# lzc452/SSL-VIT-VIDEO-ANALYTICS

Hardware: AMD Instinct MI355X
Metric: clips/sec (8x3x224x224) MAE ViT-Tiny pretrain, 1/2/4/8 GPU + recon-loss parity (higher is better)
Workload: dtype bf16; 1 GPU; BASELINE config 2: TinyViT-21M-variant MAE (stem+stages 1-3) + 4x384 decoder, T=8, 224x224, mask 0.75, bf16 autocast; model=tiny_vit_21m_variant + TinyVideoMAE, global_batch=256, per_gpu_batch=256, frames=8, image_size=224, parallelism=dp1

## Files before the change

include/sm_api.h:

```cpp
#ifndef SM_API_H
#define SM_API_H
#include <stdint.h>
#include <hip/hip_runtime_api.h>

#ifdef __cplusplus
extern "C" {
#endif

int64_t sm_gemm_workspace_bytes(int ab_dtype, int M, int N, int K);
int sm_gemm(int ab_dtype, int c_dtype, int a_layout, int b_layout, int M, int N, int K,
            const void* A, int64_t lda, const void* B, int64_t ldb, void* C, int64_t ldc,
            const float* bias, float alpha, float beta, int epi, void* aux, const void* R,
            float drop_p, uint64_t seed, const float* row_scale, int64_t rows_per_group,
            void* workspace, int64_t ws_bytes, hipStream_t stream);
int sm_gemm_persistent(int mode);
int sm_gemm_tuning(int key, int set, int value, int* prev);
int64_t sm_linear_dw_bias_workspace_bytes(int rows, int nout, int nin);
int sm_linear_dw_bias(int rows, int nout, int nin, const void* dy, const void* x, float* dW, float* db,
                      int accumulate, void* ws, int64_t ws_bytes, hipStream_t stream);
int sm_linear_dx_gelu(int M, int N, int K, const void* dy, const void* w, const void* pre, void* dx, void* h,
                      float drop_p, uint64_t seed, hipStream_t stream);
int sm_linear_dw_bias_gelu(int rows, int nout, int nin, const void* dy, const void* pre, float drop_p,
                           uint64_t seed, float* dW, float* db, int accumulate, void* ws, int64_t ws_bytes,
                           hipStream_t stream);
// ... 7 lines not shown
int sm_linear_bnin(int M, int N, int K, const void* a, const float* a_mean, const float* a_rstd,
                   const float* a_w, const float* a_b, const void* w, void* y, hipStream_t stream);
int sm_linear_bnin_bn_stats(int M, int N, int K, const void* a, const float* a_mean, const float* a_rstd,
                            const float* a_w, const float* a_b, const void* w, void* y, float* mean,
                            float* rstd, float* run_mean, float* run_var, int64_t* num_batches_tracked,
                            float momentum, float eps, int updates, void* ws, int64_t ws_bytes,
                            hipStream_t stream);
int sm_bn_apply_res_bn(int x_dtype, int y_dtype, int64_t M, int C, const void* x, const float* mean,
                       const float* rstd, const float* w, const float* b, void* y, int gelu, const void* R,
                       const float* r_mean, const float* r_rstd, const float* r_w, const float* r_b,
                       const float* row_scale, int64_t rows_per_group, hipStream_t st);
int64_t sm_linear_dw_se_workspace_bytes(int rows, int nout, int nin);
int sm_linear_dw_se(int rows, int nout, int nin, const void* dy, const void* a2, const float* act_mean,
                    const float* act_rstd, const float* act_w, const float* act_b, int act_gelu, const float* gate,
                    int hw, float* dW, int accumulate, void* ws, int64_t ws_bytes, hipStream_t stream);

int sm_attn_fwd(int dtype, int N, int L, int H, int D, const void* qkv, void* out, float* lse,
                float scale, float drop_p, uint64_t seed, hipStream_t st);
int64_t sm_attn_bwd_workspace_bytes(int dtype, int N, int L, int H, int D);
int sm_attn_bwd(int dtype, int N, int L, int H, int D, const void* qkv, const void* o,
                const void* dout, const float* lse, float* delta_ws, void* dqkv,
                float scale, float drop_p, uint64_t seed, hipStream_t st);
int sm_attn_tuning(int key, int set, int value, int* prev);

int sm_layernorm_fwd(int x_dtype, int y_dtype, int64_t M, int C, const void* x, const float* gamma,
                     const float* beta, void* y, float* mean, float* rstd, float eps, hipStream_t st);
int64_t sm_layernorm_bwd_workspace_bytes(int64_t M, int C);
int sm_layernorm_bwd(int x_dtype, int dy_dtype, int dx_dtype, int64_t M, int C, const void* dy,
                     const void* x, const float* mean, const float* rstd, const float* gamma,
                     void* dx, const void* dres, float* dgamma, float* dbeta, void* ws,
// ... 74 lines not shown
                        const float* w, void* y, float* part, hipStream_t st);
int64_t sm_dwconv_fused_bwd_workspace_bytes(int F, int H, int W, int C, int stride);
int sm_dwconv_fused_bwd(int F, int H, int W, int C, int stride, const void* dy, const void* x,
                        const float* in_mean, const float* in_rstd, const float* in_w, const float* in_b,
                        int in_gelu, const float* w, void* dx, float* dw, void* ws, int64_t ws_bytes,
                        hipStream_t st);
int64_t sm_dwconv_bn_bwd_workspace_bytes(int F, int H, int W, int C);
int sm_dwconv_bn_bwd(int F, int H, int W, int C, const void* dy, const void* x, const float* bn_mean,
                     const float* bn_rstd, const float* bn_w, const float* bn_b, int bn_gelu, const float* w,
                     void* dx, float* dw, float* dgamma, float* dbeta, void* ws, int64_t ws_bytes,
                     hipStream_t st);
int sm_dwconv_s2_bn_bwd(int F, int H, int W, int C, const void* dy, const void* x, const float* bn_mean,
                        const float* bn_rstd, const float* bn_w, const float* bn_b, int bn_gelu, const float* w,
                        void* dx, float* dw, float* dgamma, float* dbeta, void* ws, int64_t ws_bytes,
                        hipStream_t st);
int sm_dwconv_bwd(int dtype, const void* dy, const void* x, const float* w, void* dx, float* dw, int F,
                  int H, int W, int C, int stride, void* ws, int64_t ws_bytes, hipStream_t st);

int64_t sm_se_workspace_bytes(int F, int HW, int C);
int sm_se_fwd(int dtype, const void* x, const float* act_mean, const float* act_rstd, const float* act_w,
              const float* act_b, int act_gelu, int F, int HW, int C, int R, const float* w1, const float* w2,
              float* pooled, float* z1, float* s, void* y, void* ws, int64_t ws_bytes, hipStream_t st);
int sm_se_bwd(int dtype, const void* dy, const void* x, const float* act_mean, const float* act_rstd,
              const float* act_w, const float* act_b, int act_gelu, int F, int HW, int C, int R,
              const float* w1, const float* w2, const float* s, const float* z1, float* dz2, float* dz1,
              void* dx, void* ws, int64_t ws_bytes, hipStream_t st);
int sm_se_scale(int dtype, const void* x, const float* act_mean, const float* act_rstd, const float* act_w,
                const float* act_b, int act_gelu, const float* s, void* y, int F, int HW, int C, hipStream_t st);
int64_t sm_se_bn_bwd_workspace_bytes(int F, int HW, int C);
int sm_se_bn_bwd(int dtype, const void* dy, const void* x, const float* bn_mean, const float* bn_rstd,
// ... 52 lines not shown
```

ssl-vit-video-analytics_amd/csrc/conv.hip:

```cpp
#include <algorithm>

#include "common.h"
#include "sm_api.h"

namespace {

inline int ew_blocks(int64_t n) {
  int64_t b = (n + 255) / 256;
  if (b > 16384) b = 16384;
  return b < 1 ? 1 : (int)b;
}

struct ClipView {
  const float* p;
  int B, T, H, W;
  int64_t sB, sC, sT, sH, sW;
};

template <typename TO>
__global__ void stem_im2col_kernel(ClipView v, int Ho, int Wo, int stride, TO* col ) {
  const int64_t P = (int64_t)v.B * v.T * Ho * Wo;
  for (int64_t i = blockIdx.x * (int64_t)blockDim.x + threadIdx.x; i < P; i += (int64_t)gridDim.x * blockDim.x) {
    const int xo = (int)(i % Wo);
    const int64_t r = i / Wo;
// ... 1852 lines not shown
  else
    hipLaunchKernelGGL((dwf_wgrad_kernel<2>), g2, dim3(256), lds, st, (const __bf16*)dy, (const __bf16*)x, act, part,
                       H, W, C, Ho, Wo, dwf_remap());
  colred(part, F, C * 9, nullptr, dw, 1, st);
  SM_CHECK_LAUNCH();
  return 0;
}

extern "C" int64_t sm_dwconv_bn_bwd_workspace_bytes(int F, int H, int W, int C) {
  return ((int64_t)F * C * 9 + (int64_t)F * 2 * C + 2 * C) * 4 + 2 * C * 8 + 64;
}

static int dwconv_bn_bwd(int stride, int F, int H, int W, int C, const void* dy, const void* x, const float* bn_mean,
                         const float* bn_rstd, const float* bn_w, const float* bn_b, int bn_gelu, const float* w,
                         void* dx, float* dw, float* dgamma, float* dbeta, void* ws, int64_t ws_bytes,
                         hipStream_t st) {
  if (bad_stride(stride)) return -2;
  const int Ho = (H + 2 - 3) / stride + 1, Wo = (W + 2 - 3) / stride + 1;
  size_t lds = stride == 1 ? dwf_lds_bytes(W, 1) + DWB_PAD + 4 * DWF_CB * 4
                           : (size_t)DwRing<1, DWB2_TYO>::NR * (Wo + 2) * 64 + DWB2_PAD + 13 * DWF_CB * 4;
  if (lds < 256 * 4 * 4) lds = 256 * 4 * 4;
  if (!dwf_shape_ok(F, W, C, stride) || !bn_mean || !dx || lds > 64 * 1024) return -2;
  if (stride == 2 && DwRing<1, DWB2_TYO>::NEW * Wo * 4 > 256 * DWF_KV) return -2;
  if (((uintptr_t)x & 15) || ((uintptr_t)dy & 15) || ((uintptr_t)dx & 15) || C / 8 > 256) return -2;
  if (ws_bytes < sm_dwconv_bn_bwd_workspace_bytes(F, H, W, C)) return -4;
  float* part_w = (float*)ws;
  float* part_bn = part_w + (int64_t)F * C * 9;
  float* coef = part_bn + (int64_t)F * 2 * C;
  double* sums = (double*)(((uintptr_t)(coef + 2 * C) + 7) & ~(uintptr_t)7);
  ChanAffine bn{bn_mean, bn_rstd, bn_w, bn_b, bn_gelu};
  const dim3 grid((C / DWF_CB) * F);
  if (stride == 2) {
    const bool rag = W % DWB2_PX != 0;
    if (bn_gelu && !rag)
      hipLaunchKernelGGL((dwb2_kernel<true, false>), grid, dim3(256), lds, st, (const __bf16*)dy, (const __bf16*)x, bn,
                         w, (__bf16*)dx, part_w, part_bn, H, W, C, Ho, Wo, dwf_remap());
    else if (bn_gelu)
      hipLaunchKernelGGL((dwb2_kernel<true, true>), grid, dim3(256), lds, st, (const __bf16*)dy, (const __bf16*)x, bn,
                         w, (__bf16*)dx, part_w, part_bn, H, W, C, Ho, Wo, dwf_remap());
    else
      hipLaunchKernelGGL((dwb2_kernel<false, true>), grid, dim3(256), lds, st, (const __bf16*)dy, (const __bf16*)x, bn,
                         w, (__bf16*)dx, part_w, part_bn, H, W, C, Ho, Wo, dwf_remap());
  } else {
    if (bn_gelu)
      hipLaunchKernelGGL((dwb_kernel<true, true>), grid, dim3(256), lds, st, (const __bf16*)dy, (const __bf16*)x, bn,
                         w, (__bf16*)dx, part_w, part_bn, H, W, C, dwf_remap());
    else
      hipLaunchKernelGGL((dwb_kernel<false, true>), grid, dim3(256), lds, st, (const __bf16*)dy, (const __bf16*)x, bn,
                         w, (__bf16*)dx, part_w, part_bn, H, W, C, dwf_remap());
  }
  colred(part_w, F, C * 9, nullptr, dw, 1, st);
  colred(part_bn, F, 2 * C, sums, nullptr, 0, st);
  const int64_t M = (int64_t)F * H * W;
  hipLaunchKernelGGL(se_bn_finalize_kernel, dim3((C + 127) / 128), dim3(128), 0, st, sums, M, C, dgamma, dbeta,
                     coef);
  int64_t rpb = (M + 4095) / 4096;
  if (rpb < 16) rpb = 16;
  hipLaunchKernelGGL(dwb_dx_kernel, dim3((unsigned)((M + rpb - 1) / rpb)), dim3(256), 0, st, (const __bf16*)x, bn,
                     (const float*)coef, (__bf16*)dx, M, C, (int)rpb);
  SM_CHECK_LAUNCH();
  return 0;
}

extern "C" int sm_dwconv_bn_bwd(int F, int H, int W, int C, const void* dy, const void* x, const float* bn_mean,
                                const float* bn_rstd, const float* bn_w, const float* bn_b, int bn_gelu,
                                const float* w, void* dx, float* dw, float* dgamma, float* dbeta, void* ws,
                                int64_t ws_bytes, hipStream_t st) {
  return dwconv_bn_bwd(1, F, H, W, C, dy, x, bn_mean, bn_rstd, bn_w, bn_b, bn_gelu, w, dx, dw, dgamma, dbeta, ws,
                       ws_bytes, st);
}

extern "C" int sm_dwconv_s2_bn_bwd(int F, int H, int W, int C, const void* dy, const void* x, const float* bn_mean,
                                   const float* bn_rstd, const float* bn_w, const float* bn_b, int bn_gelu,
                                   const float* w, void* dx, float* dw, float* dgamma, float* dbeta, void* ws,
                                   int64_t ws_bytes, hipStream_t st) {
  return dwconv_bn_bwd(2, F, H, W, C, dy, x, bn_mean, bn_rstd, bn_w, bn_b, bn_gelu, w, dx, dw, dgamma, dbeta, ws,
                       ws_bytes, st);
}

extern "C" int64_t sm_dwconv_wgrad_workspace_bytes(int F, int H, int W, int C, int stride) {
  if (bad_stride(stride)) return 0;
  const int Ho = (H + 2 - 3) / stride + 1, Wo = (W + 2 - 3) / stride + 1;
  const int64_t P = (int64_t)F * Ho * Wo;
  int64_t ppb = (P + 1023) / 1024;
  if (ppb < 64) ppb = 64;
  const int64_t nb = (P + ppb - 1) / ppb;
  return nb * C * 9 * 4;
}

extern "C" int sm_dwconv_bwd(int dtype, const void* dy, const void* x, const float* w, void* dx, float* dw, int F,
                             int H, int W, int C, int stride, void* ws, int64_t ws_bytes, hipStream_t st) {
  if (C % 8 || C / 8 > 256) return -2;
// ... 118 lines not shown
```

ssl-vit-video-analytics_amd/csrc/gemm.hip:

```cpp
#include "common.h"
#include "sm_api.h"
#include <stdlib.h>

namespace {

struct GemmArgs {
  int M, N, K;
  int k_begin, k_chunk;
  const void* A; int64_t lda;
  const void* B; int64_t ldb;
  void* C; int64_t ldc;
  const float* bias;
  float alpha, beta;
  int epi;
  void* aux;
  const void* R;
  float drop_p;
  uint64_t seed;
  const float* row_scale;
  int64_t rows_per_group;
  float* partial;
  float* colsum;
  int cH, cW, cC, cflip;
  float xb_p;
  uint64_t xb_seed;
  ChanAffine xb_act;
  const float* xb_gate;
  int xb_hw;
  float* stat_part;
  int ctrans;
  void* aux_out;
};

template <typename TC>
SM_DEV void epilogue_store(const GemmArgs& g, int64_t row, int col, float acc, int zs) {
  if (g.partial) {
    g.partial[(int64_t)zs * g.M * g.N + row * g.N + col] = acc;
    return;
  }
  float v = g.alpha * acc;
  if (g.bias) v += g.bias[col];
  TC* C = (TC*)g.C;
  const int64_t idx = g.ctrans ? (int64_t)col * g.ldc + row : row * g.ldc + col;
  if (g.epi & 2) v = (float)(__bf16)v;
  if (g.epi & 4) v *= gelu_grad(to_f<TC>(((const TC*)g.aux)[idx]));
  if (g.epi & 1) {
// ... 758 lines not shown
  TileLoader<BNV, NT, BK> tlb;
  ConvRowsA<BMV, NT> cla;
  ConvColsB<BNV, NT> clb;
  XformColsB<BNV, NT, IMP> xlb;
  if constexpr (IMP == 1 || IMP == 10) cla.init(g, m0, kb);
  else tla.init(g.lda, g.M - m0);
  if constexpr (IMP == 2) clb.init(g, n0, kb);
  else if constexpr (XB) xlb.init(g, n0);
  else tlb.init(g.ldb, g.N - n0);

  const int64_t abase = AK ? (int64_t)m0 * g.lda : (int64_t)m0;
  const int64_t bbase = BK ? (int64_t)n0 * g.ldb : (int64_t)n0;
  const int64_t astep = AK ? 1 : g.lda, bstep = BK ? 1 : g.ldb;
  const int64_t cbase = -(int64_t)(g.cW + 1) * g.cC;
  auto load_a = [&](int k0, uint4 (&r)[TileLoader<BMV, NT, AK>::CH]) {
    if constexpr (IMP == 1 || IMP == 10) cla.load(panel_rsrc(A, (int64_t)m0 * g.cC + cbase), g, ke, r);
    else tla.load(panel_rsrc(A, abase + k0 * astep), ke - k0, r);
  };
  auto load_b = [&](int k0, uint4 (&r)[TileLoader<BNV, NT, BK>::CH]) {
    if constexpr (IMP == 2) clb.load(panel_rsrc(B, (int64_t)k0 * g.cC + cbase), g, ke - k0, r);
    else if constexpr (XB) xlb.load(g, n0, k0, ke - k0);
    else tlb.load(panel_rsrc(B, bbase + k0 * bstep), ke - k0, r);
  };

  f32x16 acc[2][NJ];
#pragma unroll
  for (int i = 0; i < 2; ++i)
#pragma unroll
    for (int j = 0; j < NJ; ++j)
#pragma unroll
      for (int r = 0; r < 16; ++r) acc[i][j][r] = 0.f;

// ... 1135 lines not shown
  if (M <= 0 || K <= 0) return 0;
  if (N <= 0 || N % 8 || K % 8 || (((uintptr_t)dy | (uintptr_t)w | (uintptr_t)pre | (uintptr_t)dx | (uintptr_t)h) & 15))
    return -2;
  GemmArgs g{};
  g.M = M; g.N = K; g.K = N; g.A = dy; g.lda = N; g.B = w; g.ldb = K; g.C = dx; g.ldc = K;
  g.alpha = 1.f; g.beta = 0.f; g.epi = 4; g.aux = const_cast<void*>(pre); g.aux_out = h;
  g.drop_p = drop_p; g.seed = seed; g.rows_per_group = 1; g.k_begin = 0; g.k_chunk = N;
  const int v = gemm_variant(g.M, g.N, g.K);
  const int tiles = ((g.N + 127) / 128) * ((g.M + variant_bm(v) - 1) / variant_bm(v));
  if (v == 2 && pp_ok_gelu_bwd(g) && launch_pp<false, 9>(g, stream)) {
    SM_CHECK_LAUNCH();
    return 0;
  }
  if (v == 2) hipLaunchKernelGGL((gemm_bf16_v2<true, false, __bf16, true, 256, 9>), dim3(tiles), dim3(512), 0, stream, g);
  else hipLaunchKernelGGL((gemm_bf16_v2<true, false, __bf16, true, 128, 9>), dim3(tiles), dim3(256), 0, stream, g);
  SM_CHECK_LAUNCH();
  return 0;
}

extern "C" int sm_gemm(int ab_dtype, int c_dtype, int a_layout, int b_layout, int M, int N, int K,
                       const void* A, int64_t lda, const void* B, int64_t ldb, void* C, int64_t ldc,
                       const float* bias, float alpha, float beta, int epi, void* aux, const void* R,
                       float drop_p, uint64_t seed, const float* row_scale, int64_t rows_per_group,
                       void* workspace, int64_t ws_bytes, hipStream_t stream) {
  return gemm_run(ab_dtype, c_dtype, a_layout, b_layout, M, N, K, A, lda, B, ldb, C, ldc, bias, alpha, beta, epi,
                  aux, R, drop_p, seed, row_scale, rows_per_group, workspace, ws_bytes, nullptr, nullptr, stream);
}

extern "C" int64_t sm_colsum_workspace_bytes(int64_t M, int C);
extern "C" int sm_colsum(int dtype, int64_t M, int C, const void* x, float* out, int accumulate, void* ws,
// ... 304 lines not shown
```

ssl-vit-video-analytics_amd/ssl_mae_amd/_lib.py:

```python
import ctypes
import os

import torch

_HERE = os.path.dirname(os.path.abspath(__file__))
LIB_PATH = os.environ.get("SM_LIB_PATH") or os.path.join(_HERE, "libsslmae.so")

F32, BF16 = 0, 1
_DT = {torch.float32: F32, torch.bfloat16: BF16}

_c_i32 = ctypes.c_int
_c_i64 = ctypes.c_int64
_c_f32 = ctypes.c_float
_c_u64 = ctypes.c_uint64
_c_p = ctypes.c_void_p

_SIGS = {
    "sm_gemm_workspace_bytes": (_c_i64, [_c_i32, _c_i32, _c_i32, _c_i32]),
    "sm_gemm_persistent": (_c_i32, [_c_i32]),
    "sm_gemm_tuning": (_c_i32, [_c_i32, _c_i32, _c_i32, _c_p]),
    "sm_attn_tuning": (_c_i32, [_c_i32, _c_i32, _c_i32, _c_p]),
    "sm_calibrate_mfma": (_c_i32, [_c_i32, _c_i32, _c_i32, _c_p, _c_p, _c_p]),
    "sm_gemm": (_c_i32, [_c_i32, _c_i32, _c_i32, _c_i32, _c_i32, _c_i32, _c_i32, _c_p, _c_i64, _c_p, _c_i64,
                         _c_p, _c_i64, _c_p, _c_f32, _c_f32, _c_i32, _c_p, _c_p, _c_f32, _c_u64, _c_p, _c_i64,
# ... 65 lines not shown
    "sm_conv3x3_wgrad": (_c_i32, [_c_p, _c_p, _c_p] + [_c_i32] * 6 + [_c_p, _c_i64, _c_p]),
    "sm_conv_wunpack_add": (_c_i32, [_c_p, _c_p, _c_i32, _c_i32, _c_i32, _c_i32, _c_p]),
    "sm_se_workspace_bytes": (_c_i64, [_c_i32, _c_i32, _c_i32]),
    "sm_se_fwd": (_c_i32, [_c_i32, _c_p] + [_c_p] * 4 + [_c_i32] * 5 + [_c_p] * 7 + [_c_i64, _c_p]),
    "sm_se_bwd": (_c_i32, [_c_i32, _c_p, _c_p] + [_c_p] * 4 + [_c_i32] * 5 + [_c_p] * 8 + [_c_i64, _c_p]),
    "sm_se_scale": (_c_i32, [_c_i32, _c_p] + [_c_p] * 4 + [_c_i32, _c_p, _c_p, _c_i32, _c_i32, _c_i32, _c_p]),
    "sm_se_bn_bwd_workspace_bytes": (_c_i64, [_c_i32, _c_i32, _c_i32]),
    "sm_se_bn_bwd": (_c_i32, [_c_i32, _c_p, _c_p] + [_c_p] * 4 + [_c_i32] * 5 + [_c_p] * 9 + [_c_p, _c_i64, _c_p]),
    "sm_dwconv_fused_partial_rows": (_c_i64, [_c_i32, _c_i32, _c_i32]),
    "sm_dwconv_fused_fwd": (_c_i32, [_c_i32] * 5 + [_c_p] * 5 + [_c_i32] + [_c_p] * 4),
    "sm_dwconv_fused_bwd_workspace_bytes": (_c_i64, [_c_i32] * 5),
    "sm_dwconv_fused_bwd": (_c_i32, [_c_i32] * 5 + [_c_p] * 6 + [_c_i32] + [_c_p] * 4 + [_c_i64, _c_p]),
    "sm_dwconv_bn_bwd_workspace_bytes": (_c_i64, [_c_i32] * 4),
    "sm_dwconv_bn_bwd": (_c_i32, [_c_i32] * 4 + [_c_p] * 6 + [_c_i32] + [_c_p] * 6 + [_c_i64, _c_p]),
    "sm_dwconv_s2_bn_bwd": (_c_i32, [_c_i32] * 4 + [_c_p] * 6 + [_c_i32] + [_c_p] * 6 + [_c_i64, _c_p]),
    "sm_bn_eval_params": (_c_i32, [_c_p, _c_p, _c_i32, _c_f32, _c_p, _c_p, _c_p]),
    "sm_segment_mean": (_c_i32, [_c_i32, _c_p, _c_i32, _c_i32, _c_i32, _c_p, _c_p]),
    "sm_segment_mean_bwd": (_c_i32, [_c_i32, _c_p, _c_i32, _c_i32, _c_i32, _c_p, _c_p]),
    "sm_bn_partials_workspace_bytes": (_c_i64, [_c_i32]),
    "sm_bn_stats_from_partials": (_c_i32, [_c_p, _c_i64, _c_i32, _c_i64] + [_c_p] * 5 + [_c_f32, _c_f32, _c_i32,
                                                                                       _c_p, _c_i64, _c_p]),
    "sm_dwconv_fwd": (_c_i32, [_c_i32, _c_p, _c_p, _c_p, _c_i32, _c_i32, _c_i32, _c_i32, _c_i32, _c_p]),
    "sm_dwconv_wgrad_workspace_bytes": (_c_i64, [_c_i32, _c_i32, _c_i32, _c_i32, _c_i32]),
    "sm_dwconv_bwd": (_c_i32, [_c_i32, _c_p, _c_p, _c_p, _c_p, _c_p, _c_i32, _c_i32, _c_i32, _c_i32, _c_i32, _c_p,
                               _c_i64, _c_p]),
    "sm_tube_mask": (_c_i32, [_c_p, _c_i32, _c_i32, _c_i32, _c_i32, _c_p, _c_p, _c_p]),
    "sm_pos_blend_fwd": (_c_i32, [_c_i32, _c_i32, _c_p, _c_p, _c_p, _c_p, _c_p, _c_p, _c_i32, _c_i32, _c_i32,
                                  _c_i32, _c_p]),
    "sm_pos_blend_bwd": (_c_i32, [_c_i32, _c_i32, _c_p, _c_p, _c_p, _c_p, _c_p, _c_p, _c_p, _c_i32, _c_i32, _c_i32,
                                  _c_i32, _c_p]),
# ... 74 lines not shown
```

ssl-vit-video-analytics_amd/ssl_mae_amd/functions.py:

```python
import math

import torch

from . import ops as K


class Mode:
    __slots__ = ("bf16", "act", "seed_base")

    def __init__(self, bf16, seed_base=0):
        self.bf16 = bool(bf16)
        self.act = torch.bfloat16 if bf16 else torch.float32
        self.seed_base = int(seed_base)

    def seed(self, module_index, site):
        return splitmix64(self.seed_base ^ splitmix64((module_index << 8) | site))


_M64 = (1 << 64) - 1


def splitmix64(x):
    x = (x + 0x9E3779B97F4A7C15) & _M64
    x = ((x ^ (x >> 30)) * 0xBF58476D1CE4E5B9) & _M64
# ... 232 lines not shown
        del da3
        if ctx.fused:
            da2, dz2, dz1 = K.se_bn_bwd(dh3, a2, Fr, Ho * Wo, mid, w_fc0.detach(), w_fc2.detach(), gate, h1se,
                                        act2, G(g2), G(b2))
        else:
            dh2, dz2, dz1 = K.se_bwd(dh3, h2, Fr, Ho * Wo, mid, w_fc0.detach(), w_fc2.detach(), gate, h1se)
            del h2
            da2 = K.bn_bwd(dh2, a2, m2, r2, g2.detach(), b2.detach(), True, G(g2), G(b2))
            del dh2
        del dh3
        R = mid // 4
        K.gemm(dz2, h1se, G(w_fc2), mid, R, Fr, 1, 1, mid, R, R, beta=1.0)
        K.gemm(dz1, pooled, G(w_fc0), R, mid, Fr, 1, 1, R, mid, mid, beta=1.0)
        if a1 is None:
            a1 = expand(x)
        if ctx.fused:
            act0 = (m0, r0, g0.detach(), b0.detach(), True)
            da1 = K.dwconv_bn_bwd(da2, a1, act0, w_dw.detach().view(mid, 9), G(w_dw).view(mid, 9), G(g0), G(b0),
                                  Fr, H, Wd, mid, stride=s)
            dh1 = None
        else:
            h1 = K.bn_apply(a1, m0, r0, g0.detach(), b0.detach(), gelu=True)
            dh1 = K.dwconv_bwd(da2, h1, w_dw.detach().view(mid, 9), G(w_dw).view(mid, 9), Fr, H, Wd, mid, s)
            del h1
        del da2
        if dh1 is not None:
            da1 = K.bn_bwd(dh1, a1, m0, r0, g0.detach(), b0.detach(), True, G(g0), G(b0))
            del dh1
        x2d = x.reshape(-1, Cin)
        if xbn is not None:
            K.linear_dw_se(da1, x2d, xbn, None, 0, G(w_exp).view(mid, Cin))
        else:
            K.linear_dw(da1, x2d, G(w_exp).view(mid, Cin))
        dx = K.linear_dx(da1, W(w_exp, mode).view(mid, Cin), residual=dout2d if st.res else None)
        _done(*ctx.params)
        return (dx.view(Fr, H, Wd, Cin),) + (None,) * 12


class BlockFn(torch.autograd.Function):

    @staticmethod
    def forward(ctx, x, st, ln1w, ln1b, wqkv, bqkv, wproj, bproj, ln2w, ln2b, w1, b1, w2, b2):
        mode = st.mode
        act = mode.act
# ... 173 lines not shown
```

ssl-vit-video-analytics_amd/ssl_mae_amd/kernels.py:

```python
import math

import torch

from . import _lib
from ._lib import call, dt, ptr, query, stream


def _chk(*ts):
    for t in ts:
        if t is not None and not t.is_cuda:
            raise _lib.KernelError("ssl_mae_amd kernels need device tensors (no CPU fallback)")


def _ws(nbytes, device):
    return torch.empty(max(int(nbytes), 16), dtype=torch.uint8, device=device)


def gemm(A, B, C, M, N, K, a_layout, b_layout, lda, ldb, ldc, bias=None, alpha=1.0, beta=0.0,
         gelu=False, aux=None, R=None, round_branch=False, drop_p=0.0, seed=0, row_scale=None, rows_per_group=1,
         gelu_bwd=False):
    _chk(A, B, C)
    ab = dt(A)
    if dt(B) != ab:
        raise _lib.KernelError("GEMM operands must share a dtype")
# ... 572 lines not shown
         ptr(dw_sink), ptr(ws), nbytes, stream())
    return dx


def dwconv_bn_bwd(dy, x, act, w, dw_sink, dg_sink, db_sink, F, H, W, C, stride=1):
    _chk(dy, x)
    dx = torch.empty_like(x)
    nbytes = query("sm_dwconv_bn_bwd_workspace_bytes", F, H, W, C)
    ws = _ws(nbytes, x.device)
    a = _act_args(act)
    call("sm_dwconv_s2_bn_bwd" if stride == 2 else "sm_dwconv_bn_bwd", F, H, W, C, ptr(dy), ptr(x), a[0], a[1], a[2], a[3], a[4], ptr(w), ptr(dx),
         ptr(dw_sink), ptr(dg_sink), ptr(db_sink), ptr(ws), nbytes, stream())
    return dx


def se_fwd(x, F, HW, C, w1, w2, act=None, want_y=True):
    R = w1.shape[0]
    dev = x.device
    pooled = torch.empty((F, C), dtype=torch.float32, device=dev)
    h1 = torch.empty((F, R), dtype=torch.float32, device=dev)
    s = torch.empty((F, C), dtype=torch.float32, device=dev)
    y = torch.empty_like(x) if want_y else None
    nbytes = query("sm_se_workspace_bytes", F, HW, C)
    ws = _ws(nbytes, dev)
    call("sm_se_fwd", dt(x), ptr(x), *_act_args(act), F, HW, C, R, ptr(w1), ptr(w2), ptr(pooled), ptr(h1), ptr(s),
         ptr(y), ptr(ws), nbytes, stream())
    return y, pooled, h1, s


def se_scale(x, s, F, HW, C, act=None):
# ... 201 lines not shown
```

ssl-vit-video-analytics_amd/ssl_mae_amd/ops.py:

```python
import torch

from . import kernels as _K

_M64 = (1 << 64) - 1


def _s64(seed):
    u = int(seed) & _M64
    return u - (1 << 64) if u >= (1 << 63) else u


def _u64(s):
    return int(s) & _M64


def _op(name, schema, mutates=()):
    def deco(impl):
        return torch.library.custom_op(f"ssl_mae::{name}", impl, mutates_args=tuple(mutates), schema=schema)
    return deco


def _none(*a, **k):
    return None

# ... 716 lines not shown

@_op("dwconv_bn_bwd", "(Tensor dy, Tensor x, Tensor bn_mean, Tensor bn_rstd, Tensor bn_w, Tensor bn_b, "
                      "bool bn_gelu, Tensor w, Tensor(a!) dw_sink, Tensor(b!) dg_sink, Tensor(c!) db_sink, int F, "
                      "int H, int W, int C, int stride=1) -> Tensor", ("dw_sink", "dg_sink", "db_sink"))
def _dwconv_bn_bwd(dy, x, bm, br, bw, bb, bg, w, dw_sink, dg_sink, db_sink, F, H, W, C, stride=1):
    return _K.dwconv_bn_bwd(dy, x, (bm, br, bw, bb, bg), w, dw_sink, dg_sink, db_sink, F, H, W, C, stride)


_dwconv_bn_bwd.register_fake(lambda dy, x, *a: torch.empty_like(x))


def dwconv_bn_bwd(dy, x, act, w, dw_sink, dg_sink, db_sink, F, H, W, C, stride=1):
    return torch.ops.ssl_mae.dwconv_bn_bwd(dy, x, *_act(act), w, dw_sink, dg_sink, db_sink, F, H, W, C, int(stride))


@_op("se_fwd", "(Tensor x, int F, int HW, int C, Tensor w1, Tensor w2, Tensor? act_mean, Tensor? act_rstd, "
               "Tensor? act_w, Tensor? act_b, bool act_gelu) -> (Tensor, Tensor, Tensor, Tensor)")
def _se_fwd(x, F, HW, C, w1, w2, am, ar, aw, ab, ag):
    act = None if am is None else (am, ar, aw, ab, ag)
    return _K.se_fwd(x, F, HW, C, w1, w2, act=act)


@_se_fwd.register_fake
def _(x, F, HW, C, w1, w2, *a):
    R = w1.shape[0]
    f = torch.float32
    return torch.empty_like(x), x.new_empty((F, C), dtype=f), x.new_empty((F, R), dtype=f), x.new_empty((F, C), dtype=f)


def se_fwd(x, F, HW, C, w1, w2, act=None):
# ... 407 lines not shown
```

Baseline: 199.1 clips/s.

## Fold expand-conv BatchNorm backward into weight and dx GEMMs algebraically

In the MBConv backward pass, the BN0 input-gradient pass over the large mid-channel activation is no longer materialized. The dwconv backward now emits the pre-BN gradient dz and the BN coefficients. A prep kernel builds a stacked folded weight and bias, and dx is computed by one two-operand GEMM over [dz, x] with K concatenated. The expand-weight gradient is rebuilt from dz^T x, a Cin×Cin Gram matrix of x and column sums, which removes a full elementwise BN-backward pass and its memory traffic. This adds small per-channel fp64 prep kernels, an extra GEMM over x, and some numerical risk from the reformulation.

Result: faster. 203.3 clips/s, median of 6 (+2.1%).

```diff
diff --git a/include/sm_api.h b/include/sm_api.h
--- a/include/sm_api.h
+++ b/include/sm_api.h
@@ -45,6 +45,14 @@
 int sm_linear_dw_se(int rows, int nout, int nin, const void* dy, const void* a2, const float* act_mean,
                     const float* act_rstd, const float* act_w, const float* act_b, int act_gelu, const float* gate,
                     int hw, float* dW, int accumulate, void* ws, int64_t ws_bytes, hipStream_t stream);
+int sm_linear_dx2(int M, int N, int K1, int K2, const void* a1, int64_t lda1, const void* a2, int64_t lda2,
+                  const void* w, const float* bias, const void* residual, void* dx, hipStream_t stream);
+int sm_mbconv_fold_prep(int mid, int Cin, const float* coef, const float* bn_mean, const float* bn_rstd,
+                        const float* bn_w, const void* w, const float* x_mean, const float* x_rstd,
+                        const float* x_w, const float* x_b, void* wst, float* r0, float* vec, hipStream_t st);
+int sm_mbconv_fold_dw(int mid, int Cin, int64_t M, const float* vec, const void* w, const float* P, const float* G,
+                      const float* s, const float* x_mean, const float* x_rstd, const float* x_w, const float* x_b,
+                      float* dW, hipStream_t st);
 
 int sm_attn_fwd(int dtype, int N, int L, int H, int D, const void* qkv, void* out, float* lse,
                 float scale, float drop_p, uint64_t seed, hipStream_t st);
@@ -149,6 +157,10 @@
                         const float* bn_rstd, const float* bn_w, const float* bn_b, int bn_gelu, const float* w,
                         void* dx, float* dw, float* dgamma, float* dbeta, void* ws, int64_t ws_bytes,
                         hipStream_t st);
+int sm_dwconv_bn_bwd_dz(int stride, int F, int H, int W, int C, const void* dy, const void* x, const float* bn_mean,
+                        const float* bn_rstd, const float* bn_w, const float* bn_b, int bn_gelu, const float* w,
+                        void* dz, float* dw, float* dgamma, float* dbeta, float* coef, void* ws, int64_t ws_bytes,
+                        hipStream_t st);
 int sm_dwconv_bwd(int dtype, const void* dy, const void* x, const float* w, void* dx, float* dw, int F,
                   int H, int W, int C, int stride, void* ws, int64_t ws_bytes, hipStream_t st);
 
diff --git a/ssl-vit-video-analytics_amd/csrc/conv.hip b/ssl-vit-video-analytics_amd/csrc/conv.hip
--- a/ssl-vit-video-analytics_amd/csrc/conv.hip
+++ b/ssl-vit-video-analytics_amd/csrc/conv.hip
@@ -1890,7 +1890,7 @@
 static int dwconv_bn_bwd(int stride, int F, int H, int W, int C, const void* dy, const void* x, const float* bn_mean,
                          const float* bn_rstd, const float* bn_w, const float* bn_b, int bn_gelu, const float* w,
                          void* dx, float* dw, float* dgamma, float* dbeta, void* ws, int64_t ws_bytes,
-                         hipStream_t st) {
+                         hipStream_t st, float* coef_out = nullptr) {
   if (bad_stride(stride)) return -2;
   const int Ho = (H + 2 - 3) / stride + 1, Wo = (W + 2 - 3) / stride + 1;
   size_t lds = stride == 1 ? dwf_lds_bytes(W, 1) + DWB_PAD + 4 * DWF_CB * 4
@@ -1904,6 +1904,7 @@
   float* part_bn = part_w + (int64_t)F * C * 9;
   float* coef = part_bn + (int64_t)F * 2 * C;
   double* sums = (double*)(((uintptr_t)(coef + 2 * C) + 7) & ~(uintptr_t)7);
+  if (coef_out) coef = coef_out;
   ChanAffine bn{bn_mean, bn_rstd, bn_w, bn_b, bn_gelu};
   const dim3 grid((C / DWF_CB) * F);
   if (stride == 2) {
@@ -1930,6 +1931,10 @@
   const int64_t M = (int64_t)F * H * W;
   hipLaunchKernelGGL(se_bn_finalize_kernel, dim3((C + 127) / 128), dim3(128), 0, st, sums, M, C, dgamma, dbeta,
                      coef);
+  if (coef_out) {
+    SM_CHECK_LAUNCH();
+    return 0;
+  }
   int64_t rpb = (M + 4095) / 4096;
   if (rpb < 16) rpb = 16;
   hipLaunchKernelGGL(dwb_dx_kernel, dim3((unsigned)((M + rpb - 1) / rpb)), dim3(256), 0, st, (const __bf16*)x, bn,
@@ -1952,6 +1957,15 @@
                                    int64_t ws_bytes, hipStream_t st) {
   return dwconv_bn_bwd(2, F, H, W, C, dy, x, bn_mean, bn_rstd, bn_w, bn_b, bn_gelu, w, dx, dw, dgamma, dbeta, ws,
                        ws_bytes, st);
+}
+
+extern "C" int sm_dwconv_bn_bwd_dz(int stride, int F, int H, int W, int C, const void* dy, const void* x,
+                                   const float* bn_mean, const float* bn_rstd, const float* bn_w, const float* bn_b,
+                                   int bn_gelu, const float* w, void* dz, float* dw, float* dgamma, float* dbeta,
+                                   float* coef, void* ws, int64_t ws_bytes, hipStream_t st) {
+  if (!coef) return -2;
+  return dwconv_bn_bwd(stride, F, H, W, C, dy, x, bn_mean, bn_rstd, bn_w, bn_b, bn_gelu, w, dz, dw, dgamma, dbeta, ws,
+                       ws_bytes, st, coef);
 }
 
 extern "C" int64_t sm_dwconv_wgrad_workspace_bytes(int F, int H, int W, int C, int stride) {
diff --git a/ssl-vit-video-analytics_amd/csrc/gemm.hip b/ssl-vit-video-analytics_amd/csrc/gemm.hip
--- a/ssl-vit-video-analytics_amd/csrc/gemm.hip
+++ b/ssl-vit-video-analytics_amd/csrc/gemm.hip
@@ -30,6 +30,9 @@
   float* stat_part;
   int ctrans;
   void* aux_out;
+  const void* A2;
+  int64_t lda2;
+  int k1;
 };
 
 template <typename TC>
@@ -818,8 +821,18 @@
   const int64_t astep = AK ? 1 : g.lda, bstep = BK ? 1 : g.ldb;
   const int64_t cbase = -(int64_t)(g.cW + 1) * g.cC;
   auto load_a = [&](int k0, uint4 (&r)[TileLoader<BMV, NT, AK>::CH]) {
-    if constexpr (IMP == 1 || IMP == 10) cla.load(panel_rsrc(A, (int64_t)m0 * g.cC + cbase), g, ke, r);
-    else tla.load(panel_rsrc(A, abase + k0 * astep), ke - k0, r);
+    if constexpr (IMP == 1 || IMP == 10) {
+      cla.load(panel_rsrc(A, (int64_t)m0 * g.cC + cbase), g, ke, r);
+    } else if constexpr (IMP == 14) {
+      if (k0 < g.k1) {
+        tla.load(panel_rsrc(A, abase + k0), g.k1 - k0, r);
+      } else {
+        if (k0 == g.k1) tla.init(g.lda2, g.M - m0);
+        tla.load(panel_rsrc((const __bf16*)g.A2, (int64_t)m0 * g.lda2 + (k0 - g.k1)), ke - k0, r);
+      }
+    } else {
+      tla.load(panel_rsrc(A, abase + k0 * astep), ke - k0, r);
+    }
   };
   auto load_b = [&](int k0, uint4 (&r)[TileLoader<BNV, NT, BK>::CH]) {
     if constexpr (IMP == 2) clb.load(panel_rsrc(B, (int64_t)k0 * g.cC + cbase), g, ke - k0, r);
@@ -1985,6 +1998,26 @@
   }
   if (v == 2) hipLaunchKernelGGL((gemm_bf16_v2<true, false, __bf16, true, 256, 9>), dim3(tiles), dim3(512), 0, stream, g);
   else hipLaunchKernelGGL((gemm_bf16_v2<true, false, __bf16, true, 128, 9>), dim3(tiles), dim3(256), 0, stream, g);
+  SM_CHECK_LAUNCH();
+  return 0;
+}
+
+extern "C" int sm_linear_dx2(int M, int N, int K1, int K2, const void* a1, int64_t lda1, const void* a2, int64_t lda2,
+                             const void* w, const float* bias, const void* residual, void* dx, hipStream_t stream) {
+  if (M <= 0 || N <= 0) return 0;
+  if (K1 <= 0 || K1 % BKT || K2 <= 0 || K2 % 8 || N % 8 || lda1 < K1 || lda2 < K2 || lda1 % 8 || lda2 % 8 ||
+      a1 == nullptr || a2 == nullptr || w == nullptr || dx == nullptr ||
+      (((uintptr_t)a1 | (uintptr_t)a2 | (uintptr_t)w | (uintptr_t)dx | (uintptr_t)residual) & 15))
+    return -2;
+  GemmArgs g{};
+  g.M = M; g.N = N; g.K = K1 + K2; g.A = a1; g.lda = lda1; g.B = w; g.ldb = N; g.C = dx; g.ldc = N;
+  g.A2 = a2; g.lda2 = lda2; g.k1 = K1;
+  g.bias = bias; g.alpha = 1.f; g.beta = residual ? 1.f : 0.f; g.R = residual;
+  g.rows_per_group = 1; g.k_begin = 0; g.k_chunk = g.K;
+  const int v = gemm_variant(M, N, g.K) == 2 ? 2 : 3;
+  const int tiles = ((N + 127) / 128) * ((M + variant_bm(v) - 1) / variant_bm(v));
+  if (v == 2) hipLaunchKernelGGL((gemm_bf16_v2<true, false, __bf16, true, 256, 14>), dim3(tiles), dim3(512), 0, stream, g);
+  else hipLaunchKernelGGL((gemm_bf16_v2<true, false, __bf16, true, 128, 14>), dim3(tiles), dim3(256), 0, stream, g);
   SM_CHECK_LAUNCH();
   return 0;
 }
diff --git a/ssl-vit-video-analytics_amd/csrc/mbfold.hip b/ssl-vit-video-analytics_amd/csrc/mbfold.hip
--- /dev/null
+++ b/ssl-vit-video-analytics_amd/csrc/mbfold.hip
@@ -0,0 +1,125 @@
+#include "common.h"
+
+namespace {
+
+constexpr int MBF_MAXMID = 2048, MBF_MAXCIN = 1024;
+
+__global__ __launch_bounds__(256) void mbconv_fold_prep_kernel(int mid, int Cin, const float* coef, const float* mean,
+                                                               const float* rstd, const float* gamma, const __bf16* W,
+                                                               ChanAffine xbn, __bf16* wst, float* r0, float* vec) {
+  __shared__ float tab[MBF_MAXMID];
+  const int b = blockIdx.x, t = threadIdx.x;
+  if (b < mid) {
+    const float rho = rstd[b], om = gamma[b] * rho, k1 = coef[mid + b];
+    for (int j = t; j < Cin; j += 256) wst[(int64_t)b * Cin + j] = (__bf16)(om * (float)W[(int64_t)b * Cin + j]);
+    if (t == 0) {
+      vec[b] = om;
+      vec[mid + b] = om * rho * k1;
+      vec[2 * mid + b] = om * (rho * k1 * mean[b] - coef[b]);
+    }
+    return;
+  }
+  for (int c = t; c < mid; c += 256) {
+    const float rho = rstd[c];
+    tab[c] = gamma[c] * rho * rho * coef[mid + c];
+  }
+  __syncthreads();
+  if (b < mid + Cin) {
+    const int i = b - mid;
+    const float sc = xbn.mean ? xbn.rstd[i] * xbn.w[i] : 1.f;
+    for (int j = t; j < Cin; j += 256) {
+      float acc = 0.f;
+      for (int c = 0; c < mid; ++c) acc = fmaf(tab[c] * (float)W[(int64_t)c * Cin + i], (float)W[(int64_t)c * Cin + j], acc);
+      wst[(int64_t)b * Cin + j] = (__bf16)(-sc * acc);
+    }
+    return;
+  }
+  for (int c = t; c < mid; c += 256) {
+    double u = 0.0;
+    if (xbn.mean)
+      for (int i = 0; i < Cin; ++i) {
+        const float sci = xbn.rstd[i] * xbn.w[i];
+        u += (double)bn_shift(xbn.b[i], xbn.mean[i], sci) * (double)(float)W[(int64_t)c * Cin + i];
+      }
+    const float rho = rstd[c], om = gamma[c] * rho;
+    const double cc = (double)om * ((double)rho * coef[mid + c] * mean[c] - (double)coef[c]);
+    tab[c] = (float)(cc - (double)tab[c] * u);
+  }
+  __syncthreads();
+  for (int j = t; j < Cin; j += 256) {
+    double acc = 0.0;
+    for (int c = 0; c < mid; ++c) acc += (double)tab[c] * (double)(float)W[(int64_t)c * Cin + j];
+    r0[j] = (float)acc;
+  }
+}
+
+__global__ __launch_bounds__(256) void mbconv_fold_dw_kernel(int mid, int Cin, double M, const float* vec,
+                                                             const __bf16* W, const float* P, const float* G,
+                                                             const float* s, ChanAffine xbn, float* dW) {
+  __shared__ float wa[MBF_MAXCIN];
+  __shared__ double red[2][256];
+  const int c = blockIdx.x, t = threadIdx.x;
+  double a1 = 0.0, a2 = 0.0;
+  for (int i = t; i < Cin; i += 256) {
+    const float w = (float)W[(int64_t)c * Cin + i];
+    const float sc = xbn.mean ? xbn.rstd[i] * xbn.w[i] : 1.f;
+    wa[i] = w * sc;
+    a1 += (double)wa[i] * (double)s[i];
+    if (xbn.mean) a2 += (double)w * (double)bn_shift(xbn.b[i], xbn.mean[i], sc);
+  }
+  red[0][t] = a1;
+  red[1][t] = a2;
+  __syncthreads();
+  a1 = a2 = 0.0;
+  for (int q = 0; q < 256; ++q) {
+    a1 += red[0][q];
+    a2 += red[1][q];
+  }
+  const double om = vec[c], dl = vec[mid + c], cc = vec[2 * mid + c];
+  for (int j = t; j < Cin; j += 256) {
+    double wg = 0.0;
+    for (int i = 0; i < Cin; ++i) wg += (double)wa[i] * (double)G[(int64_t)i * Cin + j];
+    double sj = s[j];
+    if (xbn.mean) {
+      const float sc = xbn.rstd[j] * xbn.w[j];
+      const double sh = bn_shift(xbn.b[j], xbn.mean[j], sc);
+      sj = (double)sc * sj + M * sh;
+      wg = (double)sc * wg + a1 * sh + a2 * sj;
+    }
+    const int64_t e = (int64_t)c * Cin + j;
+    dW[e] += (float)(om * (double)P[e] + cc * sj - dl * wg);
+  }
+}
+
+bool xbn_ok(const float* m, const float* r, const float* w, const float* b) {
+  return (m == nullptr) == (r == nullptr) && (m == nullptr) == (w == nullptr) && (m == nullptr) == (b == nullptr);
+}
+
+}
+
+extern "C" int sm_mbconv_fold_prep(int mid, int Cin, const float* coef, const float* bn_mean, const float* bn_rstd,
+                                   const float* bn_w, const void* w, const float* x_mean, const float* x_rstd,
+                                   const float* x_w, const float* x_b, void* wst, float* r0, float* vec,
+                                   hipStream_t st) {
+  if (mid <= 0 || Cin <= 0 || mid > MBF_MAXMID || Cin > MBF_MAXCIN || !coef || !bn_mean || !bn_rstd || !bn_w || !w ||
+      !wst || !r0 || !vec || !xbn_ok(x_mean, x_rstd, x_w, x_b))
+    return -2;
+  ChanAffine xbn{x_mean, x_rstd, x_w, x_b, 0};
+  hipLaunchKernelGGL(mbconv_fold_prep_kernel, dim3(mid + Cin + 1), dim3(256), 0, st, mid, Cin, coef, bn_mean, bn_rstd,
+                     bn_w, (const __bf16*)w, xbn, (__bf16*)wst, r0, vec);
+  SM_CHECK_LAUNCH();
+  return 0;
+}
+
+extern "C" int sm_mbconv_fold_dw(int mid, int Cin, int64_t M, const float* vec, const void* w, const float* P,
+                                 const float* G, const float* s, const float* x_mean, const float* x_rstd,
+                                 const float* x_w, const float* x_b, float* dW, hipStream_t st) {
+  if (mid <= 0 || Cin <= 0 || mid > MBF_MAXMID || Cin > MBF_MAXCIN || M <= 0 || !vec || !w || !P || !G || !s || !dW ||
+      !xbn_ok(x_mean, x_rstd, x_w, x_b))
+    return -2;
+  ChanAffine xbn{x_mean, x_rstd, x_w, x_b, 0};
+  hipLaunchKernelGGL(mbconv_fold_dw_kernel, dim3(mid), dim3(256), 0, st, mid, Cin, (double)M, vec, (const __bf16*)w, P,
+                     G, s, xbn, dW);
+  SM_CHECK_LAUNCH();
+  return 0;
+}
diff --git a/ssl-vit-video-analytics_amd/ssl_mae_amd/_lib.py b/ssl-vit-video-analytics_amd/ssl_mae_amd/_lib.py
--- a/ssl-vit-video-analytics_amd/ssl_mae_amd/_lib.py
+++ b/ssl-vit-video-analytics_amd/ssl_mae_amd/_lib.py
@@ -103,6 +103,10 @@
     "sm_dwconv_bn_bwd_workspace_bytes": (_c_i64, [_c_i32] * 4),
     "sm_dwconv_bn_bwd": (_c_i32, [_c_i32] * 4 + [_c_p] * 6 + [_c_i32] + [_c_p] * 6 + [_c_i64, _c_p]),
     "sm_dwconv_s2_bn_bwd": (_c_i32, [_c_i32] * 4 + [_c_p] * 6 + [_c_i32] + [_c_p] * 6 + [_c_i64, _c_p]),
+    "sm_dwconv_bn_bwd_dz": (_c_i32, [_c_i32] * 5 + [_c_p] * 6 + [_c_i32] + [_c_p] * 7 + [_c_i64, _c_p]),
+    "sm_linear_dx2": (_c_i32, [_c_i32] * 4 + [_c_p, _c_i64, _c_p, _c_i64] + [_c_p] * 5),
+    "sm_mbconv_fold_prep": (_c_i32, [_c_i32, _c_i32] + [_c_p] * 13),
+    "sm_mbconv_fold_dw": (_c_i32, [_c_i32, _c_i32, _c_i64] + [_c_p] * 11),
     "sm_bn_eval_params": (_c_i32, [_c_p, _c_p, _c_i32, _c_f32, _c_p, _c_p, _c_p]),
     "sm_segment_mean": (_c_i32, [_c_i32, _c_p, _c_i32, _c_i32, _c_i32, _c_p, _c_p]),
     "sm_segment_mean_bwd": (_c_i32, [_c_i32, _c_p, _c_i32, _c_i32, _c_i32, _c_p, _c_p]),
diff --git a/ssl-vit-video-analytics_amd/ssl_mae_amd/functions.py b/ssl-vit-video-analytics_amd/ssl_mae_amd/functions.py
--- a/ssl-vit-video-analytics_amd/ssl_mae_amd/functions.py
+++ b/ssl-vit-video-analytics_amd/ssl_mae_amd/functions.py
@@ -3,6 +3,8 @@
 import torch
 
 from . import ops as K
+
+BN0_FOLD = True
 
 
 class Mode:
@@ -270,6 +272,23 @@
         K.gemm(dz1, pooled, G(w_fc0), R, mid, Fr, 1, 1, R, mid, mid, beta=1.0)
         if a1 is None:
             a1 = expand(x)
+        x2d = x.reshape(-1, Cin)
+        if ctx.fused and BN0_FOLD and mid % 64 == 0 and Cin % 8 == 0 and Cin <= mid // 2:
+            act0 = (m0, r0, g0.detach(), b0.detach(), True)
+            dz, coef = K.dwconv_bn_bwd_dz(da2, a1, act0, w_dw.detach().view(mid, 9), G(w_dw).view(mid, 9), G(g0),
+                                          G(b0), Fr, H, Wd, mid, stride=s)
+            del da2, a1
+            wb = W(w_exp, mode).view(mid, Cin)
+            wst, r0f, vec = K.mbconv_fold_prep(coef, m0, r0, g0.detach(), wb)
+            xf = x2d if xbn is None else K.bn_apply(x2d, *xbn[:4], gelu=False)
+            P = K.linear_dw(dz, xf, torch.empty((mid, Cin), dtype=torch.float32, device=dz.device), accumulate=False)
+            gram = torch.zeros((Cin, Cin), dtype=torch.float32, device=dz.device)
+            xsum = torch.zeros(Cin, dtype=torch.float32, device=dz.device)
+            K.linear_dw_bias(xf, xf, gram, xsum)
+            K.mbconv_fold_dw(vec, wb, P, gram, xsum, xf.shape[0], G(w_exp).view(mid, Cin))
+            dx = K.linear_dx2(dz, xf, wst, bias=r0f, residual=dout2d if st.res else None)
+            _done(*ctx.params)
+            return (dx.view(Fr, H, Wd, Cin),) + (None,) * 12
         if ctx.fused:
             act0 = (m0, r0, g0.detach(), b0.detach(), True)
             da1 = K.dwconv_bn_bwd(da2, a1, act0, w_dw.detach().view(mid, 9), G(w_dw).view(mid, 9), G(g0), G(b0),
@@ -283,7 +302,6 @@
         if dh1 is not None:
             da1 = K.bn_bwd(dh1, a1, m0, r0, g0.detach(), b0.detach(), True, G(g0), G(b0))
             del dh1
-        x2d = x.reshape(-1, Cin)
         if xbn is not None:
             K.linear_dw_se(da1, x2d, xbn, None, 0, G(w_exp).view(mid, Cin))
         else:
diff --git a/ssl-vit-video-analytics_amd/ssl_mae_amd/kernels.py b/ssl-vit-video-analytics_amd/ssl_mae_amd/kernels.py
--- a/ssl-vit-video-analytics_amd/ssl_mae_amd/kernels.py
+++ b/ssl-vit-video-analytics_amd/ssl_mae_amd/kernels.py
@@ -610,6 +610,62 @@
     return dx
 
 
+def dwconv_bn_bwd_dz(dy, x, act, w, dw_sink, dg_sink, db_sink, F, H, W, C, stride=1):
+    _chk(dy, x)
+    dz = torch.empty_like(x)
+    coef = torch.empty((2, C), dtype=torch.float32, device=x.device)
+    nbytes = query("sm_dwconv_bn_bwd_workspace_bytes", F, H, W, C)
+    ws = _ws(nbytes, x.device)
+    a = _act_args(act)
+    call("sm_dwconv_bn_bwd_dz", int(stride), F, H, W, C, ptr(dy), ptr(x), a[0], a[1], a[2], a[3], a[4], ptr(w),
+         ptr(dz), ptr(dw_sink), ptr(dg_sink), ptr(db_sink), ptr(coef), ptr(ws), nbytes, stream())
+    return dz, coef
+
+
+def _xbn_args(xbn):
+    return [None] * 4 if xbn is None else [ptr(t) for t in xbn[:4]]
+
+
+def mbconv_fold_prep(coef, mean, rstd, gamma, w, xbn=None):
+    _chk(coef, mean, rstd, gamma, w)
+    mid, Cin = w.shape
+    if w.dtype != torch.bfloat16 or not w.is_contiguous() or tuple(coef.shape) != (2, mid):
+        raise _lib.KernelError("mbconv_fold_prep: contiguous bf16 w [mid, Cin], coef [2, mid]")
+    wst = torch.empty((mid + Cin, Cin), dtype=torch.bfloat16, device=w.device)
+    r0 = torch.empty(Cin, dtype=torch.float32, device=w.device)
+    vec = torch.empty((3, mid), dtype=torch.float32, device=w.device)
+    call("sm_mbconv_fold_prep", mid, Cin, ptr(coef), ptr(mean), ptr(rstd), ptr(gamma), ptr(w), *_xbn_args(xbn),
+         ptr(wst), ptr(r0), ptr(vec), stream())
+    return wst, r0, vec
+
+
+def mbconv_fold_dw(vec, w, P, G, s, M, grad_sink, xbn=None):
+    _chk(vec, w, P, G, s, grad_sink)
+    mid, Cin = w.shape
+    if (tuple(P.shape) != (mid, Cin) or tuple(G.shape) != (Cin, Cin) or s.numel() != Cin
+            or tuple(grad_sink.shape) != (mid, Cin) or tuple(vec.shape) != (3, mid) or w.dtype != torch.bfloat16):
+        raise _lib.KernelError("mbconv_fold_dw: shape mismatch")
+    call("sm_mbconv_fold_dw", mid, Cin, int(M), ptr(vec), ptr(w), ptr(P), ptr(G), ptr(s), *_xbn_args(xbn),
+         ptr(grad_sink), stream())
+    return grad_sink
+
+
+def linear_dx2(a1, a2, w, bias=None, residual=None):
+    _chk(a1, a2, w, bias, residual)
+    M, K1 = a1.shape
+    K2 = a2.shape[1]
+    N = w.shape[1]
+    if (a2.shape[0] != M or w.shape[0] != K1 + K2 or a1.stride(1) != 1 or a2.stride(1) != 1 or not w.is_contiguous()
+            or any(t.dtype != torch.bfloat16 for t in (a1, a2, w))
+            or (residual is not None and (tuple(residual.shape) != (M, N) or residual.dtype != torch.bfloat16
+                                          or not residual.is_contiguous()))):
+        raise _lib.KernelError("linear_dx2: bf16 a1 [M,K1], a2 [M,K2], w [K1+K2,N], residual [M,N]")
+    dx = torch.empty((M, N), dtype=torch.bfloat16, device=a1.device)
+    call("sm_linear_dx2", M, N, K1, K2, ptr(a1), a1.stride(0), ptr(a2), a2.stride(0), ptr(w), ptr(bias),
+         ptr(residual), ptr(dx), stream())
+    return dx
+
+
 def se_fwd(x, F, HW, C, w1, w2, act=None, want_y=True):
     R = w1.shape[0]
     dev = x.device
diff --git a/ssl-vit-video-analytics_amd/ssl_mae_amd/ops.py b/ssl-vit-video-analytics_amd/ssl_mae_amd/ops.py
--- a/ssl-vit-video-analytics_amd/ssl_mae_amd/ops.py
+++ b/ssl-vit-video-analytics_amd/ssl_mae_amd/ops.py
@@ -754,6 +754,69 @@
     return torch.ops.ssl_mae.dwconv_bn_bwd(dy, x, *_act(act), w, dw_sink, dg_sink, db_sink, F, H, W, C, int(stride))
 
 
+@_op("dwconv_bn_bwd_dz", "(Tensor dy, Tensor x, Tensor bn_mean, Tensor bn_rstd, Tensor bn_w, Tensor bn_b, "
+                         "bool bn_gelu, Tensor w, Tensor(a!) dw_sink, Tensor(b!) dg_sink, Tensor(c!) db_sink, int F, "
+                         "int H, int W, int C, int stride=1) -> (Tensor, Tensor)", ("dw_sink", "dg_sink", "db_sink"))
+def _dwconv_bn_bwd_dz(dy, x, bm, br, bw, bb, bg, w, dw_sink, dg_sink, db_sink, F, H, W, C, stride=1):
+    return _K.dwconv_bn_bwd_dz(dy, x, (bm, br, bw, bb, bg), w, dw_sink, dg_sink, db_sink, F, H, W, C, stride)
+
+
+_dwconv_bn_bwd_dz.register_fake(lambda dy, x, *a: (torch.empty_like(x),
+                                                   x.new_empty((2, x.shape[-1]), dtype=torch.float32)))
+
+
+def dwconv_bn_bwd_dz(dy, x, act, w, dw_sink, dg_sink, db_sink, F, H, W, C, stride=1):
+    return torch.ops.ssl_mae.dwconv_bn_bwd_dz(dy, x, *_act(act), w, dw_sink, dg_sink, db_sink, F, H, W, C,
+                                              int(stride))
+
+
+def _xbn(xbn):
+    return (None,) * 4 if xbn is None else tuple(xbn[:4])
+
+
+@_op("mbconv_fold_prep", "(Tensor coef, Tensor bn_mean, Tensor bn_rstd, Tensor bn_w, Tensor w, Tensor? x_mean, "
+                         "Tensor? x_rstd, Tensor? x_w, Tensor? x_b) -> (Tensor, Tensor, Tensor)")
+def _mbconv_fold_prep(coef, bm, br, bw, w, xm, xr, xw, xb):
+    return _K.mbconv_fold_prep(coef, bm, br, bw, w, None if xm is None else (xm, xr, xw, xb))
+
+
+@_mbconv_fold_prep.register_fake
+def _(coef, bm, br, bw, w, *a):
+    mid, cin = w.shape
+    return (w.new_empty((mid + cin, cin)), w.new_empty(cin, dtype=torch.float32),
+            w.new_empty((3, mid), dtype=torch.float32))
+
+
+def mbconv_fold_prep(coef, mean, rstd, gamma, w, xbn=None):
+    return torch.ops.ssl_mae.mbconv_fold_prep(coef, mean, rstd, gamma, w, *_xbn(xbn))
+
+
+@_op("mbconv_fold_dw", "(Tensor vec, Tensor w, Tensor P, Tensor G, Tensor s, int M, Tensor(a!) grad_sink, "
+                       "Tensor? x_mean, Tensor? x_rstd, Tensor? x_w, Tensor? x_b) -> ()", ("grad_sink",))
+def _mbconv_fold_dw(vec, w, P, G, s, M, grad_sink, xm, xr, xw, xb):
+    _K.mbconv_fold_dw(vec, w, P, G, s, M, grad_sink, None if xm is None else (xm, xr, xw, xb))
+
+
+_mbconv_fold_dw.register_fake(_none)
+
+
+def mbconv_fold_dw(vec, w, P, G, s, M, grad_sink, xbn=None):
+    torch.ops.ssl_mae.mbconv_fold_dw(vec, w, P, G, s, int(M), grad_sink, *_xbn(xbn))
+    return grad_sink
+
+
+@_op("linear_dx2", "(Tensor a1, Tensor a2, Tensor w, Tensor? bias, Tensor? residual) -> Tensor")
+def _linear_dx2(a1, a2, w, bias, residual):
+    return _K.linear_dx2(a1, a2, w, bias, residual)
+
+
+_linear_dx2.register_fake(lambda a1, a2, w, *a: a1.new_empty((a1.shape[0], w.shape[1])))
+
+
+def linear_dx2(a1, a2, w, bias=None, residual=None):
+    return torch.ops.ssl_mae.linear_dx2(a1, a2, w, bias, residual)
+
+
 @_op("se_fwd", "(Tensor x, int F, int HW, int C, Tensor w1, Tensor w2, Tensor? act_mean, Tensor? act_rstd, "
                "Tensor? act_w, Tensor? act_b, bool act_gelu) -> (Tensor, Tensor, Tensor, Tensor)")
 def _se_fwd(x, F, HW, C, w1, w2, am, ar, aw, ab, ag):
```
